# alexoz12v2/cuda-optix-pathtracing

Measured on AMD Instinct MI355X. Metric: Msamples/s (paths x spp / s), higher is better.
Workload: dtype f32

## Files before the change

### cuda-optix-pathtracing_amd/binding.py

```python
import ctypes as C
import subprocess
from pathlib import Path

import numpy as np

_HERE = Path(__file__).resolve().parent
_CSRC = _HERE / "csrc"
_LIB = None

DMT_ACCEL_BRUTE_FORCE = 0
DMT_ACCEL_BVH = 1
BVH_BUILD_HOST = 0
BVH_BUILD_DEVICE = 1
BVH_BUILT_BY_HOST = 0
BVH_BUILT_BY_DEVICE = 1
BVH_BUILT_BY_HOST_AFTER_DEVICE = 2
BVH_UPDATE_REBUILD = 0
BVH_UPDATE_REFIT = 1
BVH_UPDATE_AUTO = 2
BVH_UPDATED_NONE = 0
BVH_UPDATED_REFIT = 1
BVH_UPDATED_REBUILD = 2
BVH_UPDATED_REBUILD_AFTER_REFIT = 3

# ... 30 lines not shown
    return _LIB


EXPORTED_SYMBOLS = [
    "dmt_ctx_create", "dmt_ctx_destroy", "dmt_last_error", "dmt_upload_triangles", "dmt_upload_bsdfs",
    "dmt_upload_lights", "dmt_set_camera", "dmt_set_limits", "dmt_set_accel", "dmt_set_light_sampling", "dmt_light_tree_pmfs", "dmt_light_tree_ref_select", "dmt_set_bvh_strategy", "dmt_set_partition", "dmt_set_chunk", "dmt_render_profile",
    "dmt_upload_area_lights", "dmt_upload_textures", "dmt_upload_envmap", "dmt_clear_envmap", "dmt_envmap_tables", "dmt_test_envmap",
    "dmt_set_stream", "dmt_film_clear", "dmt_film_bind", "dmt_film_device_ptrs", "dmt_download_film",
    "dmt_render", "dmt_render_adaptive", "dmt_render_stats", "dmt_sync", "dmt_sched_diag", "dmt_kernel_time", "dmt_kernel_info", "dmt_bvh_validate", "dmt_brute_cull_plan", "dmt_brute_cull_box_plan", "dmt_brute_cull_box_records", "dmt_cull_box_test", "dmt_test_triangle_intersect",
    "dmt_test_sampler", "dmt_test_camera_rays", "dmt_test_bsdf", "dmt_test_bsdf_ng", "dmt_test_material", "dmt_test_light", "dmt_test_half",
    "dmt_test_trace_samples", "dmt_test_trace_log", "dmt_test_closest_hit",
    "dmt_set_texture_filter", "dmt_texture_mip_chain", "dmt_texture_footprint", "dmt_test_texture_filter",
    "dmt_render_aovs", "dmt_upload_aovs", "dmt_download_aovs", "dmt_denoise_defaults", "dmt_denoise",
    "dmt_set_accel_build", "dmt_accel_build_info", "dmt_accel_download", "dmt_lbvh_reference", "dmt_bvh_check",
    "dmt_update_vertices", "dmt_update_vertices_device", "dmt_set_accel_update", "dmt_accel_update_info", "dmt_bvh_refit_reference",
    "dmt_download_aov_surface", "dmt_upload_aov_surface", "dmt_camera_project", "dmt_test_camera_project", "dmt_temporal_defaults",
    "dmt_denoise_temporal", "dmt_temporal_reset", "dmt_temporal_info", "dmt_temporal_download",
    "dmt_set_sampler_table", "dmt_sampler_table_plan", "dmt_test_sampler_table",
    "dmt_set_lens", "dmt_lens_info", "dmt_lens_rays", "dmt_focus_distance_at", "dmt_test_lens_values",
    "dmt_set_motion", "dmt_clear_motion", "dmt_set_shutter", "dmt_motion_info", "dmt_shutter_times", "dmt_motion_positions",
    "dmt_motion_bvh_validate", "dmt_test_shutter_times", "dmt_test_closest_hit_at",
    "dmt_upload_vertex_normals", "dmt_clear_vertex_normals", "dmt_vertex_normals_info", "dmt_smooth_normals",
    "dmt_test_shading_normal", "dmt_test_shading_normal_mapped",
    "dmt_upload_opacity", "dmt_clear_opacity", "dmt_opacity_info", "dmt_opacity_eval", "dmt_test_opacity", "dmt_test_closest_hit_opacity",
]

SAMPLER_TABLE_OFF = 0
SAMPLER_TABLE_AUTO = 1
SAMPLER_TABLE_FORCE = 2


class SamplerTablePlanRecord(C.Structure):
    _fields_ = [("use", C.c_uint32), ("period_width", C.c_uint32), ("period_height", C.c_uint32), ("entry_bytes", C.c_uint32),
                ("slices", C.c_uint32), ("reserved", C.c_uint32), ("slice_bytes", C.c_uint64)]


def sampler_table_plan(width, height, owned_pixels, spp, chunk_spp, budget_bytes=0, mode=SAMPLER_TABLE_AUTO):
    lib = load_library()
    rec = SamplerTablePlanRecord()
    args = [int(width), int(height), C.c_uint64(int(owned_pixels)), C.c_uint32(int(spp)), C.c_uint32(int(chunk_spp)),
            C.c_uint64(int(budget_bytes)), int(mode)]
    rc = lib.dmt_sampler_table_plan(*args, C.byref(rec), None, C.c_uint32(0))
    if rc != 0:
        raise DmtError(f"dmt_sampler_table_plan failed ({rc})")
    lens = (C.c_uint32 * max(int(rec.slices), 1))()
    rc = lib.dmt_sampler_table_plan(*args, C.byref(rec), lens, C.c_uint32(int(rec.slices)))
# ... 579 lines not shown
        pairs = np.zeros((max(info["pairs"], 1), 2), np.uint32)
        self._check(self._lib.dmt_accel_download(self._ctx, _p(nodes), C.c_size_t(nodes.shape[0]), _p(pairs), C.c_size_t(pairs.shape[0])),
                    "dmt_accel_download")
        return nodes[:info["nodes"]].copy(), pairs[:info["pairs"]].copy()

    def set_light_sampling(self, mode):
        self._check(self._lib.dmt_set_light_sampling(self._ctx, int(mode)), "dmt_set_light_sampling")

    def set_texture_filter(self, mode):
        self._check(self._lib.dmt_set_texture_filter(self._ctx, int(mode)), "dmt_set_texture_filter")

    def set_bvh_strategy(self, strategy, paths_per_pass=0):
        self._check(self._lib.dmt_set_bvh_strategy(self._ctx, int(strategy), C.c_uint64(int(paths_per_pass))), "dmt_set_bvh_strategy")

    def set_partition(self, rank, world):
        self._check(self._lib.dmt_set_partition(self._ctx, int(rank), int(world)), "dmt_set_partition")

    def set_chunk(self, samples_per_item):
        self._check(self._lib.dmt_set_chunk(self._ctx, C.c_uint32(samples_per_item)), "dmt_set_chunk")

    def set_sampler_table(self, mode, budget_bytes=0):
        self._check(self._lib.dmt_set_sampler_table(self._ctx, int(mode), C.c_uint64(int(budget_bytes))), "dmt_set_sampler_table")

    def set_stream(self, stream_ptr):
        self._check(self._lib.dmt_set_stream(self._ctx, C.c_void_p(stream_ptr)), "dmt_set_stream")

    def film_clear(self):
        self._check(self._lib.dmt_film_clear(self._ctx), "dmt_film_clear")

    def film_bind(self, mean_ptr, m2_ptr):
        self._check(self._lib.dmt_film_bind(self._ctx, C.c_void_p(mean_ptr), C.c_void_p(m2_ptr)), "dmt_film_bind")

    def film_device_ptrs(self):
        a, b = C.c_void_p(), C.c_void_p()
        self._check(self._lib.dmt_film_device_ptrs(self._ctx, C.byref(a), C.byref(b)), "dmt_film_device_ptrs")
        return a.value, b.value

    def download_film(self):
        mean = np.zeros((self.height, self.width, 4), np.float32)
        m2 = np.zeros((self.height, self.width, 4), np.float32)
        self._check(self._lib.dmt_download_film(self._ctx, _p(mean), _p(m2)), "dmt_download_film")
        return mean, m2

    def render(self, spp, sample_offset=0, region=None):
        x0, y0, x1, y1 = region if region is not None else (0, 0, self.width, self.height)
        self._check(self._lib.dmt_render(self._ctx, C.c_uint32(sample_offset), C.c_uint32(spp), int(x0), int(y0),
# ... 100 lines not shown
        self._check(self._lib.dmt_temporal_info(self._ctx, C.byref(rec)), "dmt_temporal_info")
        return {name: getattr(rec, name) for name, _ in TemporalRecord._fields_}

    def download_history(self):
        cv = np.zeros((self.height, self.width, 4), np.float32)
        ln = np.zeros((self.height, self.width), np.float32)
        self._check(self._lib.dmt_temporal_download(self._ctx, _p(cv), _p(ln)), "dmt_temporal_download")
        return cv, ln

    def test_camera_project(self, points):
        p = _f32(points).reshape(-1, 3)
        xy, depth = np.zeros((p.shape[0], 2), np.float32), np.zeros(p.shape[0], np.float32)
        self._check(self._lib.dmt_test_camera_project(self._ctx, int(p.shape[0]), _p(p), _p(xy), _p(depth)), "dmt_test_camera_project")
        return xy, depth

    def sync(self):
        self._check(self._lib.dmt_sync(self._ctx), "dmt_sync")

    def sched_diag(self, reset=False):
        out = (C.c_uint64 * 8)()
        if not hasattr(self._lib, "dmt_sched_diag"):
            return dict.fromkeys(["folds", "handed_over", "folded_for_others", "slab_stalls", "early_exits",
                                  "max_stall_ticks_10ns", "launched", "slabs_per_wave"], 0)
        self._check(self._lib.dmt_sched_diag(self._ctx, out, int(bool(reset))), "dmt_sched_diag")
        keys = ["folds", "handed_over", "folded_for_others", "slab_stalls", "early_exits", "max_stall_ticks_10ns", "launched", "slabs_per_wave"]
        return dict(zip(keys, [int(x) for x in out]))

    def kernel_time(self, reset=True):
        ms, n = C.c_double(), C.c_uint64()
        self._check(self._lib.dmt_kernel_time(self._ctx, C.byref(ms), C.byref(n), int(bool(reset))), "dmt_kernel_time")
        return ms.value, n.value

    def kernel_info(self):
        v = [C.c_int() for _ in range(5)]
        self._check(self._lib.dmt_kernel_info(self._ctx, *[C.byref(x) for x in v]), "dmt_kernel_info")
        keys = ["vgprs", "sgprs", "lds_bytes", "blocks_per_cu", "cu_count"]
        return dict(zip(keys, (x.value for x in v)))

    def test_triangle_intersect(self, xs, ys, zs, o, d):
        xs, ys, zs = _f32(xs), _f32(ys), _f32(zs)
        n = xs.size // 4
        o, d = _f32(o), _f32(d)
        hit = np.zeros(n, np.int32)
        t = np.zeros(n, np.float32)
        pos, nrm, err = (np.zeros((n, 3), np.float32) for _ in range(3))
        self._check(self._lib.dmt_test_triangle_intersect(self._ctx, _p(xs), _p(ys), _p(zs), C.c_size_t(n), _p(o),
                                                          _p(d), _p(hit), _p(t), _p(pos), _p(nrm), _p(err)),
                    "dmt_test_triangle_intersect")
        return hit, t, pos, nrm, err
# ... 153 lines not shown
```

### cuda-optix-pathtracing_amd/csrc/dmt_hip.hip

```cpp
#include <hip/hip_runtime.h>

#include <algorithm>
#include <cassert>
#include <chrono>
#include <cmath>
#include <cstddef>
#include <cstdio>
#include <cstdlib>
#include <cstring>
#include <limits>
#include <map>
#include <memory>
#include <new>
#include <string>
#include <vector>

#include "../../include/dmt_hip.h"
#include "pt_device.hpp"
#include "bvh_device.hpp"
#include "bvh_gpu_build.hpp"
#include "devbuf.hpp"
#include "envmap.hpp"
#include "light_tree.hpp"
#include "light_tree_ref.hpp"
// ... 60 lines not shown
  int maxDepth;
  int shadeThreshold;
  EnvView env;
  uint32_t const* areaOf;
  uint32_t const* areaTri;
  float const* areaLe;
  uint32_t areaCount;
  uint32_t const* texRgba;
  int32_t const* texDesc;
  uint32_t const* matTex;
  float const* triUv;
  LightTreeNode const* lightTree;
  LightTreeRefNode const* lightTreeRef;
  unsigned long long* stats;
  float texCfr[12];
  float texMinDx[3], texMinDy[3];
  float texSppScale;
  uint32_t const* texMip;
  int32_t const* texMipDesc;
  MotionView motion;
  VtxNormalRec const* vtxNormals;
  OpacityRec const* opacity;
  float opacityCutoff8;
};

typedef RenderParams const DMT_CONST_AS* KArgs;
DMT_DEV KArgs kargs_base() { return (KArgs)__builtin_amdgcn_kernarg_segment_ptr(); }
DMT_DEV KArgs kargs(KArgs p) {
  asm volatile("" : "+s"(p));
  return p;
}
DMT_DEV SceneView load_scene(KArgs k) {
  k = kargs(k);
  SceneView s;
  s.tris = k->scene.tris, s.post = k->scene.post, s.bsdfs = k->scene.bsdfs, s.lights = k->scene.lights;
  s.infLights = k->scene.infLights, s.triCount = k->scene.triCount, s.bsdfCount = k->scene.bsdfCount;
  s.lightCount = k->scene.lightCount, s.infLightCount = k->scene.infLightCount;
  return s;
}
DMT_DEV BvhView load_bvh(KArgs k) {
  k = kargs(k);
  BvhView b;
  b.nodes = k->bvh.nodes, b.pairs = k->bvh.pairs, b.overflow = k->bvh.overflow, b.overflowStride = k->bvh.overflowStride;
  return b;
}

// ... 19 lines not shown
  unsigned long long const now = __builtin_readcyclecounter();
  unsigned long long const m = __ballot(1);
  if (int(__ffsll((long long)m)) - 1 == int(threadIdx.x & 63u)) {
    uint32_t const w = threadIdx.x >> 6;
    s_sectAcc[w][i] += now - s_sectLast[w];
    s_sectLast[w] = now;
  }
#endif
}
struct PathState {
  RayPair rp;
  f3 beta, L;
  int depth;
  bool lastT;
  bool active;
  bool hasShadow;
  bool finPending;
  float smax;
  Sampler rng;
  uint32_t sidx;
  float lastPdf;
  bool lastSpecular;
};
__shared__ float s_cold[7 * kLdsThreads];
DMT_DEV void put_C(f3 v) {
  float* const c = s_cold + threadIdx.x;
  c[0 * kLdsThreads] = v.x, c[1 * kLdsThreads] = v.y, c[2 * kLdsThreads] = v.z;
}
DMT_DEV f3 get_C() {
  float const* const c = s_cold + threadIdx.x;
  return mk3(c[0 * kLdsThreads], c[1 * kLdsThreads], c[2 * kLdsThreads]);
}
DMT_DEV void put_Lfin(f3 v) {
  float* const c = s_cold + threadIdx.x;
  c[3 * kLdsThreads] = v.x, c[4 * kLdsThreads] = v.y, c[5 * kLdsThreads] = v.z;
}
DMT_DEV f3 get_Lfin() {
  float const* const c = s_cold + threadIdx.x;
  return mk3(c[3 * kLdsThreads], c[4 * kLdsThreads], c[5 * kLdsThreads]);
}
DMT_DEV void put_finIdx(uint32_t i) { s_cold[6 * kLdsThreads + threadIdx.x] = __uint_as_float(i); }
DMT_DEV uint32_t get_finIdx() { return __float_as_uint(s_cold[6 * kLdsThreads + threadIdx.x]); }
DMT_DEV f3 ray_dir(PathState const& st) { return mk3(st.rp.dx.x, st.rp.dy.x, st.rp.dz.x); }
DMT_DEV f3 ray_org(PathState const& st) { return mk3(st.rp.ox.x, st.rp.oy.x, st.rp.oz.x); }
DMT_DEV void swap_rays(PathState& st) {
  auto sw = [](v2f& p) { float const t = p.x; p.x = p.y, p.y = t; };
// ... 993 lines not shown
template <bool STATS = false>
DMT_DEV void trace_pair_bvh(KArgs k, PathState const& st, bool doC, bool doS, uint32_t gtid, int& bestTri,
                            float& bu, float& bv, bool& occluded, LaneStats* ls = nullptr) {
  BvhView const bvh = load_bvh(k);
  float bt;
  if constexpr (STATS) ls->closest += doC ? 1u : 0u, ls->shadow += doS ? 1u : 0u;
  bvh_closest<STATS>(bvh, doC, mk3(st.rp.ox.x, st.rp.oy.x, st.rp.oz.x), mk3(st.rp.dx.x, st.rp.dy.x, st.rp.dz.x),
                     gtid, bestTri, bt, bu, bv, STATS ? &ls->tc : nullptr);
  occluded = bvh_any<STATS>(bvh, doS, mk3(st.rp.ox.y, st.rp.oy.y, st.rp.oz.y),
                            mk3(st.rp.dx.y, st.rp.dy.y, st.rp.dz.y), st.smax, gtid, STATS ? &ls->tc : nullptr);
}
DMT_DEV void trace_pair_bvh_motion(KArgs k, PathState const& st, bool doC, bool doS, v2f time, uint32_t gtid, int& bestTri, float& bu,
                                   float& bv, bool& occluded, float* btOut = nullptr) {
  BvhView const bvh = load_bvh(k);
  TriPairDelta const* const delta = kargs(k)->motion.pairDelta;
  float bt;
  bvh_closest<false>(bvh, doC, mk3(st.rp.ox.x, st.rp.oy.x, st.rp.oz.x), mk3(st.rp.dx.x, st.rp.dy.x, st.rp.dz.x), gtid, bestTri, bt, bu, bv,
                     nullptr, LeafMotion{delta, time.x});
  occluded = bvh_any<false>(bvh, doS, mk3(st.rp.ox.y, st.rp.oy.y, st.rp.oz.y), mk3(st.rp.dx.y, st.rp.dy.y, st.rp.dz.y), st.smax, gtid,
                            nullptr, LeafMotion{delta, time.y});
  if (btOut) *btOut = bt;
}

template <uint32_t F, class Sink>
DMT_DEV void lane_finish(KArgs k, PathState& st, bool doC, bool doS, int bestTri, float bu, float bv, bool occluded,
                         Sink&& sink);

template <uint32_t F, class Sink>
DMT_DEV void lane_step(KArgs k, uint32_t gtid, PathState& st, Sink&& sink, LaneStats* ls = nullptr) {
  bool const doC = st.active;
  bool const doS = st.hasShadow;
  int bestTri;
  float bu, bv;
  bool occluded;
  if constexpr ((F & kFeatCutout) && (F & kFeatBvh))
    trace_pair_bvh_cut(k, st, doC, doS, gtid, bestTri, bu, bv, occluded);
  else if constexpr (F & kFeatCutout)
    trace_pair_brute_cut(k, st, doC, doS, bestTri, bu, bv, occluded);
  else if constexpr ((F & kFeatMotion) && (F & kFeatBvh))
    trace_pair_bvh_motion(k, st, doC, doS, v2f{motion_time(), motion_time_shadow()}, gtid, bestTri, bu, bv, occluded);
  else if constexpr (F & kFeatMotion)
    trace_pair_brute_motion(k, st, doC, doS, v2f{motion_time(), motion_time_shadow()}, bestTri, bu, bv, occluded);
  else if constexpr (F & kFeatBvh)
    trace_pair_bvh<(F & kFeatStats) != 0>(k, st, doC, doS, gtid, bestTri, bu, bv, occluded, ls);
  else
    trace_pair_brute(k, st, doC, doS, bestTri, bu, bv, occluded);
  sect_mark(2);
  if constexpr (F & kFeatStats) ls->bounces += (doC && bestTri >= 0 && st.depth < kargs(k)->maxDepth) ? 1u : 0u;
  lane_finish<F & ~kFeatStats>(k, st, doC, doS, bestTri, bu, bv, occluded, sink);
}

template <uint32_t F, class Sink>
DMT_DEV void lane_finish(KArgs k, PathState& st, bool doC, bool doS, int bestTri, float bu, float bv, bool occluded,
                         Sink&& sink) {
  if (doS) {
    st.hasShadow = false;
    if (st.finPending) {
      f3 Lfin = get_Lfin();
      if (!occluded) Lfin = Lfin + get_C();
      st.finPending = false;
      sink(Lfin, get_finIdx());
    } else if (!occluded) {
      st.L = st.L + get_C();
    }
  }
  sect_mark(3);
  if (doC) {
    if (path_shade<F>(k, st, bestTri, bu, bv)) {
      st.active = false;
      if (st.hasShadow) {
        put_Lfin(st.L);
        put_finIdx(st.sidx);
        st.finPending = true;
      } else {
        sink(st.L, st.sidx);
      }
    }
  }
  if constexpr (F & kFeatMotion) {
    if (st.hasShadow) motion_park_shadow();
  }
  sect_mark(10);
}

__shared__ float s_prep[15 * kLdsThreads];

struct ColdArgs {
  CameraXf cam;
  SamplerParams sp;
// ... 103 lines not shown
  uint32_t* slabBusy;
  float* stage;
  int rank, world;
};
DMT_DEV TileArgs load_tile_args(KArgs k) {
  k = kargs(k);
  TileArgs t;
  t.mean = k->mean, t.m2 = k->m2, t.counter = k->counter, t.width = k->width;
  t.x0 = k->x0, t.y0 = k->y0, t.x1 = k->x1, t.y1 = k->y1, t.tx0 = k->tx0, t.ty0 = k->ty0, t.rtx = k->rtx;
  t.numItems = k->numItems, t.subShift = k->subShift, t.sampleOffset = k->sampleOffset, t.spp = k->spp, t.rank = k->rank, t.world = k->world;
  t.chunkSpp = k->chunkSpp, t.numChunks = k->numChunks, t.link = k->link, t.slabBusy = k->slabBusy, t.stage = k->stage;
  return t;
}

__shared__ uint32_t s_desc[kLdsThreads / 64][2][8];
__shared__ int32_t s_pixbase[2 * kLdsThreads];
__shared__ uint32_t s_pixmap[2 * kLdsThreads];

constexpr uint32_t kSlotBit = 0x80000000u;
constexpr uint32_t kFoldReady = 0xFFFFFFFFu;
#ifndef DMT_SLAB_WAIT_MS
#define DMT_SLAB_WAIT_MS 250
#endif
constexpr int kSchedDiagWords = 8;

struct WaveSched {
  uint32_t cur = 0, fetched = 0;
  uint32_t alloc = 0;
  uint32_t nextUnit = 0, totalUnits = 0;
  bool exhausted = false;
  uint32_t slabFree = (1u << kSlabsPerWave) - 1u;
  uint32_t slabPend = 0;
};
enum { SD_FOLDS = 0, SD_HANDED = 1, SD_CHAINED = 2, SD_STALLS = 3, SD_EXITS = 4, SD_MAXSTALL = 5 };
DMT_DEV void sched_count(unsigned long long* D, int lane, int what, unsigned long long n = 1ull) {
  if (lane == 0) atomicAdd(&D[what], n);
}
struct LaneSched {
  bool prepared = false;
  bool prepSlot = false;
};

struct ItemGeom {
  int px0, py0;
  uint32_t rows;
  unsigned long long live;
};
DMT_DEV ItemGeom item_geom(TileArgs const& T, uint32_t item) {
  uint32_t const band = item & ((1u << T.subShift) - 1u);
  uint32_t const rows = 8u >> T.subShift;
  uint32_t j;
  unsigned long long live = ~0ull;
  KArgs const k = kargs(kargs_base());
  if (uint32_t const* const list = k->tileList) {
    j = list[item >> T.subShift];
    live = kargs(k)->tileMask[j] >> (band * rows * 8u);
  } else {
// ... 221 lines not shown
      unsigned long long* const D = kargs(Pk)->schedDiag;
      sched_count(D, lane, SD_STALLS);
      unsigned long long const t0 = __builtin_amdgcn_s_memrealtime();
      unsigned long long waited = 0;
      do {
        __builtin_amdgcn_s_sleep(64);
        slab_refresh(T, gtid, lane, W);
        waited = __builtin_amdgcn_s_memrealtime() - t0;
      } while (W.slabFree == 0u && waited <= (unsigned long long)(DMT_SLAB_WAIT_MS) * 100000ull);
      if (lane == 0) atomicMax(&D[SD_MAXSTALL], waited);
      if (W.slabFree == 0u) {
        sched_count(D, lane, SD_EXITS);
        return false;
      }
    }
  }
  return true;
}
DMT_DEV bool lane_holds(PathState const& st, LaneSched const& Ls, bool curSlot) {
  return (st.active && ((st.sidx >> 31) != 0u) == curSlot) || (Ls.prepared && Ls.prepSlot == curSlot) ||
         (st.finPending && ((get_finIdx() >> 31) != 0u) == curSlot);
}

template <bool STATS>
DMT_DEV void flush_stats(KArgs Pk, LaneStats const& ls) {
  if constexpr (STATS) {
    unsigned long long* const stats = kargs(Pk)->stats;
    atomicAdd(&stats[0], (unsigned long long)ls.samples);
    atomicAdd(&stats[1], (unsigned long long)ls.closest);
    atomicAdd(&stats[2], (unsigned long long)ls.shadow);
    atomicAdd(&stats[3], (unsigned long long)ls.tc.nodes);
    atomicAdd(&stats[4], (unsigned long long)ls.tc.tris);
    atomicAdd(&stats[5], (unsigned long long)ls.bounces);
    atomicAdd(&stats[6], (unsigned long long)ls.itNode);
    atomicAdd(&stats[7], (unsigned long long)ls.itLeaf);
    atomicAdd(&stats[8], (unsigned long long)ls.itShade);
    atomicAdd(&stats[9], (unsigned long long)ls.itOuter);
    atomicAdd(&stats[10], (unsigned long long)ls.itPrep);
    atomicAdd(&stats[11], (unsigned long long)ls.lanesLeaf);
    atomicAdd(&stats[12], (unsigned long long)ls.lanesShade);
    atomicAdd(&stats[13], (unsigned long long)ls.lanesPrep);
    atomicAdd(&stats[14], (unsigned long long)ls.tc.deadNodes);
    atomicAdd(&stats[15], (unsigned long long)ls.tc.overflowPushes);
  }
}

template <uint32_t F>
DMT_DEV void megakernel_body() {
  static_assert(!(F & kFeatBvh), "BVH kernels run megakernel_body_bvh");
  constexpr bool STATS = (F & kFeatStats) != 0;
  constexpr bool MOTION = (F & kFeatMotion) != 0;
  KArgs const Pk = kargs_base();
  LaneStats ls;
  int const lane = int(threadIdx.x) & 63;
  uint32_t const gtid = blockIdx.x * blockDim.x + threadIdx.x;
  WaveSched W;
  LaneSched Ls;
  PathState st{};
  auto sink = [&](f3 L, uint32_t sidx) { stage_sample(Pk, sidx, L); };
#if DMT_SECTION_TIMING
  if (lane == 0) s_sectLast[threadIdx.x >> 6] = __builtin_readcyclecounter();
#endif
  if constexpr (!MOTION && !(F & kFeatCutout)) cull_stage(Pk);
#if DMT_SECTION_TIMING
  if (lane < 16) s_sectAcc[threadIdx.x >> 6][lane] = 0;
  sect_mark(15);
#endif
  {
    for (;;) {
      bool const needPrep = !Ls.prepared;
      bool const starving = !st.active && needPrep;
      if (__any(starving) || __popcll(__ballot(needPrep)) >= DMT_PREP_THRESHOLD) sched_draw<MOTION>(Pk, gtid, lane, W, Ls, needPrep);
      if (W.cur == W.fetched) break;
      if (!st.active && Ls.prepared) {
        path_begin_prepared<MOTION>(st);
        Ls.prepared = false;
        if constexpr (STATS) ++ls.samples;
      }
      sect_mark(0);
      if (W.alloc != W.cur || W.nextUnit == W.totalUnits) {
        if (!__any(lane_holds(st, Ls, (W.cur & 1u) != 0u))) {
          bool const more = sched_retire(Pk, gtid, lane, W);
          sect_mark(1);
          if (!more) break;
          continue;
        }
      }
      sect_mark(1);
      lane_step<F>(Pk, gtid, st, sink, STATS ? &ls : nullptr);
    }
  }
#if DMT_SECTION_TIMING
  if (lane < 16) atomicAdd(&g_sect[lane], s_sectAcc[threadIdx.x >> 6][lane]);
#endif
  flush_stats<STATS>(Pk, ls);
}

#ifndef DMT_BVH_NODE_WEIGHT
#define DMT_BVH_NODE_WEIGHT 1
#define DMT_BVH_LEAF_WEIGHT 2
#endif
#ifndef DMT_BVH_SHADE_THRESHOLD
#define DMT_BVH_SHADE_THRESHOLD 32
#endif
#ifndef DMT_BVH_DUMMY_LDS
#define DMT_BVH_DUMMY_LDS 0
#endif
template <uint32_t F>
DMT_DEV void megakernel_body_bvh() {
  static_assert((F & kFeatBvh) != 0, "brute-force kernels run megakernel_body");
  constexpr bool STATS = (F & kFeatStats) != 0;
  constexpr bool MOTION = (F & kFeatMotion) != 0;
  KArgs const Pk = kargs_base();
// ... 313 lines not shown
  DevBuf<float> d_env;
  EnvView env{};
  DevBuf<uint32_t> d_areaOf;
  DevBuf<uint32_t> d_areaTri;
  DevBuf<float> d_areaLe;
  uint32_t areaCount = 0;
  std::vector<uint32_t> h_areaTri;
  std::vector<float> h_areaLe;
  bool haveTris = false, haveBsdfs = false, haveLights = false, haveCamera = false;
  dmt_camera cam{};
  CameraXf xf{};
  SamplerParams sp{};
  float lensR = 0.f, lensD = 1.f;
  DevBuf<float4> ownMean, ownM2;
  float4* d_mean = nullptr;
  float4* d_m2 = nullptr;
  int filmW = 0, filmH = 0;
  DevBuf<uint32_t> d_counter;
  DevBuf<uint32_t> d_sched;
  DevBuf<unsigned long long> d_schedDiag;
  unsigned long long expectedFolds = 0;
  DevBuf<unsigned long long> d_stats;
  DevBuf<float> d_stage;
  DevBuf<float4> d_samTab;
  DevBuf<float2> d_samTabJit;
  DevBuf<float2> d_samTabLens;
  int samTabMode = DMT_SAMPLER_TABLE_AUTO;
  uint64_t samTabBudget = kSamTabDefaultBudget;
  DevBuf<unsigned long long> d_adMask;
  DevBuf<uint32_t> d_adList;
  DevBuf<uint32_t> d_adCount;
  DenoiseState dn;
  uint32_t chunkSpp = 0;
  int subShift = -1;
  int maxDepth = 32;
  int accel = DMT_ACCEL_BRUTE_FORCE;
  int rank = 0, world = 1;
  int cuCount = 0;
  std::vector<std::pair<hipEvent_t, hipEvent_t>> events;
  size_t eventsUsed = 0;
  double accumMs = 0.0;
  uint64_t accumLaunches = 0;
};

namespace {

// ... 464 lines not shown
    ctx->lightTreeNodes = uint32_t(nodes.size());
    ctx->lightTreeValid = true;
    return DMT_OK;
  }
  std::vector<light_tree::Item> items;
  for (uint32_t i = 0; i < ctx->lightCount; ++i) {
    light_tree::Item it{};
    if (!light_tree::itemOf(ctx->h_lights.data() + 32 * size_t(i), i, [](uint16_t h) { return h2f_host(h); }, it))
      return fail(ctx, DMT_ERR_STATE, "light tree: only point and spot lights can be in the light list");
    items.push_back(it);
  }
  std::vector<LightTreeNode> const nodes = light_tree::build(items, &ctx->lightTreeDepth);
  if (ctx->lightTreeDepth > 60) {
    ctx->lightTreeTooDeep = true;
    return DMT_OK;
  }
  HIP_TRY(ctx, ctx->d_lightTree.assign(nodes.data(), nodes.size()));
  ctx->lightTreeNodes = uint32_t(nodes.size());
  ctx->lightTreeValid = true;
  return DMT_OK;
}

int checkErrorFlag(dmt_ctx* ctx) {
  unsigned long long folds = 0;
  HIP_TRY(ctx, hipMemcpy(&folds, ctx->d_schedDiag.get(), sizeof(folds), hipMemcpyDeviceToHost));
  if (folds != ctx->expectedFolds) {
    char msg[200];
    snprintf(msg, sizeof(msg), "in-launch ordering: %llu sample chunks were folded into the film, %llu were launched: the film is invalid",
             folds, ctx->expectedFolds);
    ctx->expectedFolds = folds;
    return fail(ctx, DMT_ERR_HIP, msg);
  }
  return DMT_OK;
}

int finishTest(dmt_ctx* ctx) {
  HIP_TRY(ctx, hipGetLastError());
  HIP_TRY(ctx, hipStreamSynchronize(ctx->stream));
  return DMT_OK;
}

}

#include "denoise_host.hpp"

static int rebuildAreaLights(dmt_ctx* ctx);

extern "C" {
// ... 31 lines not shown
  }
  ctx->stream = ctx->ownStream;
  ctx->cuCount = prop.multiProcessorCount;
  ctx->ac.blocksPerCUBvh = bpcBvh > 0 ? bpcBvh : 1;
  if (char const* e3 = std::getenv("DMT_BVH_STRATEGY")) {
    int const v = std::atoi(e3);
    ctx->bvhStrategy = v < 0 || v > 2 ? 0 : v;
  }
  if (char const* e5 = std::getenv("DMT_BVH_SHADE_THRESHOLD")) {
    int const v = std::atoi(e5);
    ctx->ac.shadeThresholdEnv = v < 1 ? 0 : (v > 64 ? 64 : v);
  }
  if (char const* e4 = std::getenv("DMT_WF_PATHS")) {
    long long const v = std::atoll(e4);
    if (v >= 4096) ctx->wfTargetPaths = size_t(v);
  }
  if (char const* e6 = std::getenv("DMT_BRUTE_CULL")) {
    int const v = std::atoi(e6);
    ctx->bruteCull = v == 0 ? 0 : v == 1 ? 1 : 2;
  }
  if (char const* e7 = std::getenv("DMT_SAMPLER_TABLE")) {
    int const v = std::atoi(e7);
    ctx->samTabMode = v == 0 ? DMT_SAMPLER_TABLE_OFF : v == 2 ? DMT_SAMPLER_TABLE_FORCE : DMT_SAMPLER_TABLE_AUTO;
  }
  if (char const* e2 = std::getenv("DMT_SUB_SHIFT")) {
    int const v = std::atoi(e2);
    ctx->subShift = v < 0 ? -1 : (v > 2 ? 2 : v);
  }
  *out = ctx.release();
  return DMT_OK;
}

int dmt_ctx_destroy(dmt_ctx* ctx) {
  if (!ctx) return DMT_ERR_INVALID;
  (void)hipSetDevice(ctx->device);
  (void)hipStreamSynchronize(ctx->stream);
  for (auto& ev : ctx->events) {
    (void)hipEventDestroy(ev.first);
    (void)hipEventDestroy(ev.second);
  }
  if (ctx->ownStream) (void)hipStreamDestroy(ctx->ownStream);
  delete ctx;
  return DMT_OK;
}

const char* dmt_last_error(const dmt_ctx* ctx) { return ctx ? ctx->err.c_str() : g_createError.c_str(); }
// ... 360 lines not shown
  SamplerTablePlan tab;
  if (!stats6 && !wavefront && !sel && !(F & kFeatMotion))
    tab = samplerTablePlan(ctx->filmW, ctx->filmH, uint64_t(ownedTiles) * 64u, spp, P.chunkSpp, ctx->samTabBudget, ctx->samTabMode,
                           ctx->lensR > 0.f ? kSamTabLensEntryBytes : kSamTabEntryBytes);

  bool const useBvh = ctx->accel == DMT_ACCEL_BVH;
  uint32_t const wavesWanted = P.numItems * P.numChunks < P.numItems ? P.numItems : P.numItems * P.numChunks;
  uint32_t blocks = uint32_t(ctx->cuCount) * uint32_t(blocksPerCu);
  uint32_t const blocksNeeded = (wavesWanted + 3) / 4;
  if (blocks > blocksNeeded) blocks = blocksNeeded;
  if (blocks == 0) blocks = 1;

  if (ctx->eventsUsed == ctx->events.size()) {
    hipEvent_t a, b;
    HIP_TRY(ctx, hipEventCreate(&a));
    HIP_TRY(ctx, hipEventCreate(&b));
    ctx->events.emplace_back(a, b);
  }
  auto& ev = ctx->events[ctx->eventsUsed];
  {
    size_t const floats = size_t(blocks) * 4u * size_t(kSlabsPerWave) * size_t(P.chunkSpp) * 192u;
    HIP_TRY(ctx, ctx->d_stage.reserve(floats));
    P.stage = ctx->d_stage.get();
  }
  uint32_t const callChunks = P.numChunks;
  uint32_t const sliceChunks = tab.use ? tab.sliceChunks : callChunks;
  size_t const busyWords = size_t(blocks) * 4u * size_t(kSlabsPerWave);
  size_t const linkWords = sliceChunks > 1 ? size_t(P.numItems) * size_t(sliceChunks) : 0;
  {
    HIP_TRY(ctx, ctx->d_sched.reserve(busyWords + linkWords));
    P.slabBusy = ctx->d_sched.get(), P.link = ctx->d_sched.get() + busyWords;
    HIP_TRY(ctx, hipMemsetAsync(ctx->d_sched.get(), 0, (busyWords + linkWords) * sizeof(uint32_t), ctx->stream));
  }
  size_t const sliceEntries = size_t(std::min<uint64_t>(uint64_t(sliceChunks) * P.chunkSpp, spp)) * tab.pw * tab.ph;
  if (tab.use) {
    HIP_TRY(ctx, ctx->d_samTab.reserve(2 * sliceEntries));
    HIP_TRY(ctx, ctx->d_samTabJit.reserve(sliceEntries));
    P.samTab = ctx->d_samTab.get(), P.samTabJit = ctx->d_samTabJit.get(), P.samTabPw = tab.pw, P.samTabPh = tab.ph;
    if (ctx->lensR > 0.f) {
      HIP_TRY(ctx, ctx->d_samTabLens.reserve(sliceEntries));
      P.samTabLens = ctx->d_samTabLens.get();
    }
  }
  HIP_TRY(ctx, hipMemsetAsync(ctx->d_counter.get(), 0, sizeof(uint32_t), ctx->stream));
  HIP_TRY(ctx, hipEventRecord(ev.first, ctx->stream));
  uint64_t const launchFolds = uint64_t(P.numItems) * P.numChunks;
// ... 197 lines not shown
  if (!ctx || !stats16) return DMT_ERR_INVALID;
  if (ctx->accel != DMT_ACCEL_BVH) return fail(ctx, DMT_ERR_STATE, "dmt_render_profile: only the BVH path has device counters");
  return renderImpl(ctx, sample_offset, spp, x0, y0, x1, y1, stats16, 16);
}

int dmt_sync(dmt_ctx* ctx) {
  if (!ctx) return DMT_ERR_INVALID;
  HIP_TRY(ctx, hipSetDevice(ctx->device));
  HIP_TRY(ctx, hipStreamSynchronize(ctx->stream));
  return checkErrorFlag(ctx);
}

int dmt_sched_diag(dmt_ctx* ctx, uint64_t* out8, int reset) {
  if (!ctx || !out8) return DMT_ERR_INVALID;
  HIP_TRY(ctx, hipSetDevice(ctx->device));
  HIP_TRY(ctx, hipStreamSynchronize(ctx->stream));
  unsigned long long d[kSchedDiagWords] = {};
  HIP_TRY(ctx, hipMemcpy(d, ctx->d_schedDiag.get(), sizeof(d), hipMemcpyDeviceToHost));
  for (int i = 0; i < 8; ++i) out8[i] = i < kSchedDiagWords ? d[i] : 0;
  out8[6] = ctx->expectedFolds;
  out8[7] = uint64_t(kSlabsPerWave);
  if (reset) {
    HIP_TRY(ctx, hipMemset(ctx->d_schedDiag.get(), 0, sizeof(d)));
    ctx->expectedFolds = 0;
  }
  return DMT_OK;
}

static int rebuildAreaLights(dmt_ctx* ctx) {
  ctx->d_areaOf.reset(), ctx->d_areaTri.reset(), ctx->d_areaLe.reset(), ctx->areaCount = 0;
  uint32_t const n = uint32_t(ctx->h_areaTri.size());
  if (n == 0 || !ctx->haveTris) return DMT_OK;
  std::vector<uint32_t> of(ctx->triCount, 0xFFFFFFFFu);
  for (uint32_t k = 0; k < n; ++k) {
    if (ctx->h_areaTri[k] >= ctx->triCount) return fail(ctx, DMT_ERR_INVALID, "area light refers to a triangle outside the uploaded soup");
    of[ctx->h_areaTri[k]] = k;
  }
  DevBuf<uint32_t> areaOf, areaTri;
  DevBuf<float> areaLe;
  HIP_TRY(ctx, areaOf.assign(of.data(), of.size()));
  HIP_TRY(ctx, areaTri.assign(ctx->h_areaTri.data(), n));
  HIP_TRY(ctx, areaLe.assign(ctx->h_areaLe.data(), 3 * size_t(n)));
  ctx->d_areaOf = std::move(areaOf), ctx->d_areaTri = std::move(areaTri), ctx->d_areaLe = std::move(areaLe);
  ctx->areaCount = n;
  return DMT_OK;
}

int dmt_upload_area_lights(dmt_ctx* ctx, const uint32_t* triangle_index, const float* radiance_rgb, uint32_t count) {
// ... 427 lines not shown
```

### include/dmt_hip.h

```cpp
#ifndef DMT_HIP_H
#define DMT_HIP_H

#include <stddef.h>
#include <stdint.h>

#ifdef __cplusplus
extern "C" {
#endif

typedef struct dmt_ctx dmt_ctx;

typedef struct dmt_camera {
  float dir[3];
  float pos[3];
  int32_t width;
  int32_t height;
  int32_t spp;
  float focal_length;
  float sensor_size;
} dmt_camera;

enum {
  DMT_OK = 0,
  DMT_ERR_INVALID = 1,
// ... 85 lines not shown
  uint32_t entry_bytes;
  uint32_t slices;
  uint32_t reserved;
  uint64_t slice_bytes;
} dmt_sampler_table_plan_record;
int dmt_sampler_table_plan(int width, int height, uint64_t owned_pixels, uint32_t spp, uint32_t chunk_spp, uint64_t budget_bytes,
                           int mode, dmt_sampler_table_plan_record* out, uint32_t* slice_spp, uint32_t slice_cap);
int dmt_set_stream(dmt_ctx* ctx, void* hip_stream);

int dmt_film_clear(dmt_ctx* ctx);
int dmt_film_bind(dmt_ctx* ctx, void* d_mean, void* d_m2);
int dmt_film_device_ptrs(dmt_ctx* ctx, void** d_mean, void** d_m2);
int dmt_download_film(dmt_ctx* ctx, float* mean4, float* m24);

int dmt_render(dmt_ctx* ctx, uint32_t sample_offset, uint32_t spp, int x0, int y0, int x1, int y1);
int dmt_render_adaptive(dmt_ctx* ctx, uint32_t min_spp, uint32_t max_spp, uint32_t step_spp, float threshold,
                        int x0, int y0, int x1, int y1, uint32_t* rounds, uint64_t* samples);
int dmt_render_stats(dmt_ctx* ctx, uint32_t sample_offset, uint32_t spp, int x0, int y0, int x1, int y1,
                     uint64_t* stats6);
int dmt_render_profile(dmt_ctx* ctx, uint32_t sample_offset, uint32_t spp, int x0, int y0, int x1, int y1,
                       uint64_t* stats16);
int dmt_sync(dmt_ctx* ctx);
int dmt_sched_diag(dmt_ctx* ctx, uint64_t* out8, int reset);
int dmt_kernel_time(dmt_ctx* ctx, double* total_ms, uint64_t* launches, int reset);
int dmt_kernel_info(dmt_ctx* ctx, int* vgprs, int* sgprs, int* lds_bytes, int* blocks_per_cu,
                    int* cu_count);

int dmt_bvh_validate(const float* xs, const float* ys, const float* zs, size_t count, int* node_count,
                     int* depth, int* max_leaf);

enum {
  DMT_BVH_BUILD_HOST = 0,
  DMT_BVH_BUILD_DEVICE = 1,
};
enum {
  DMT_BVH_BUILT_BY_HOST = 0,
  DMT_BVH_BUILT_BY_DEVICE = 1,
  DMT_BVH_BUILT_BY_HOST_AFTER_DEVICE = 2,
};
int dmt_set_accel_build(dmt_ctx* ctx, int mode);
typedef struct dmt_accel_build_record {
  int32_t builder;
  int32_t depth;
  uint32_t triangles;
  uint32_t nodes;
  uint32_t pairs;
// ... 129 lines not shown
```

Measured before the change: 5860.

## Park GGX hits in a per-wave queue and shade them in coherent batches

Adds a per-wave global-memory queue where lanes that hit GGX dielectric or conductor materials park their path state (throughput, radiance, direction, hit, sampler dims). Lanes then refill with other paths, and the parked hits are resumed together once a threshold (default 32) is reached or the slab drains. The aim is to cut divergence in the costly microfacet shading branch so that more lanes of a wave run the same BSDF code at once. In exchange it adds extra global memory traffic for the spill and refill, more ballots and bookkeeping in the scheduler loop, and a consistency check that parked and resumed counts match. Only the plain brute-force kernel variant is affected.

```diff
diff --git a/cuda-optix-pathtracing_amd/binding.py b/cuda-optix-pathtracing_amd/binding.py
--- a/cuda-optix-pathtracing_amd/binding.py
+++ b/cuda-optix-pathtracing_amd/binding.py
@@ -76,6 +76,7 @@
     "dmt_motion_bvh_validate", "dmt_test_shutter_times", "dmt_test_closest_hit_at",
     "dmt_upload_vertex_normals", "dmt_clear_vertex_normals", "dmt_vertex_normals_info", "dmt_smooth_normals",
     "dmt_test_shading_normal", "dmt_test_shading_normal_mapped",
+    "dmt_set_ggx_batch", "dmt_ggx_batch_diag",
     "dmt_upload_opacity", "dmt_clear_opacity", "dmt_opacity_info", "dmt_opacity_eval", "dmt_test_opacity", "dmt_test_closest_hit_opacity",
 ]
 
@@ -701,6 +702,14 @@
     def set_sampler_table(self, mode, budget_bytes=0):
         self._check(self._lib.dmt_set_sampler_table(self._ctx, int(mode), C.c_uint64(int(budget_bytes))), "dmt_set_sampler_table")
 
+    def set_ggx_batch(self, batch):
+        self._check(self._lib.dmt_set_ggx_batch(self._ctx, C.c_uint32(int(batch))), "dmt_set_ggx_batch")
+
+    def ggx_batch(self):
+        out = (C.c_uint64 * 5)()
+        self._check(self._lib.dmt_ggx_batch_diag(self._ctx, out), "dmt_ggx_batch_diag")
+        return int(out[4])
+
     def set_stream(self, stream_ptr):
         self._check(self._lib.dmt_set_stream(self._ctx, C.c_void_p(stream_ptr)), "dmt_set_stream")
 
@@ -847,9 +856,14 @@
         if not hasattr(self._lib, "dmt_sched_diag"):
             return dict.fromkeys(["folds", "handed_over", "folded_for_others", "slab_stalls", "early_exits",
                                   "max_stall_ticks_10ns", "launched", "slabs_per_wave"], 0)
+        ggx = (C.c_uint64 * 5)()
+        if hasattr(self._lib, "dmt_ggx_batch_diag"):
+            self._check(self._lib.dmt_ggx_batch_diag(self._ctx, ggx), "dmt_ggx_batch_diag")
         self._check(self._lib.dmt_sched_diag(self._ctx, out, int(bool(reset))), "dmt_sched_diag")
         keys = ["folds", "handed_over", "folded_for_others", "slab_stalls", "early_exits", "max_stall_ticks_10ns", "launched", "slabs_per_wave"]
-        return dict(zip(keys, [int(x) for x in out]))
+        d = dict(zip(keys, [int(x) for x in out]))
+        d.update(ggx_parked=int(ggx[0]), ggx_resumed=int(ggx[1]), ggx_shade_passes=int(ggx[2]), ggx_shaded_full=int(ggx[3]))
+        return d
 
     def kernel_time(self, reset=True):
         ms, n = C.c_double(), C.c_uint64()
diff --git a/cuda-optix-pathtracing_amd/csrc/dmt_hip.hip b/cuda-optix-pathtracing_amd/csrc/dmt_hip.hip
--- a/cuda-optix-pathtracing_amd/csrc/dmt_hip.hip
+++ b/cuda-optix-pathtracing_amd/csrc/dmt_hip.hip
@@ -106,6 +106,8 @@
   VtxNormalRec const* vtxNormals;
   OpacityRec const* opacity;
   float opacityCutoff8;
+  uint32_t ggxBatchT;
+  float* ggxQueue;
 };
 
 typedef RenderParams const DMT_CONST_AS* KArgs;
@@ -171,6 +173,7 @@
   float lastPdf;
   bool lastSpecular;
 };
+DMT_DEV bool ggx_resumed(PathState const& st) { return st.depth < 0; }
 __shared__ float s_cold[7 * kLdsThreads];
 DMT_DEV void put_C(f3 v) {
   float* const c = s_cold + threadIdx.x;
@@ -1210,17 +1213,27 @@
   if (btOut) *btOut = bt;
 }
 
-template <uint32_t F, class Sink>
+struct NoPark {};
+template <uint32_t F, class Sink, class Park = NoPark>
 DMT_DEV void lane_finish(KArgs k, PathState& st, bool doC, bool doS, int bestTri, float bu, float bv, bool occluded,
-                         Sink&& sink);
-
-template <uint32_t F, class Sink>
-DMT_DEV void lane_step(KArgs k, uint32_t gtid, PathState& st, Sink&& sink, LaneStats* ls = nullptr) {
+                         Sink&& sink, Park&& park = Park{});
+
+template <uint32_t F, class Sink, class Park = NoPark>
+DMT_DEV void lane_step(KArgs k, uint32_t gtid, PathState& st, Sink&& sink, LaneStats* ls = nullptr, Park&& park = Park{}) {
+  constexpr bool PARK = !std::is_same<typename std::decay<Park>::type, NoPark>::value;
   bool const doC = st.active;
   bool const doS = st.hasShadow;
   int bestTri;
   float bu, bv;
   bool occluded;
+  if constexpr (PARK) {
+    static_assert(F == 0, "GGX batching: the plain brute-force row only");
+    trace_pair_brute(k, st, doC && !ggx_resumed(st), doS, bestTri, bu, bv, occluded);
+    if (ggx_resumed(st)) bestTri = __float_as_int(st.rp.ox.x), bu = st.rp.oy.x, bv = st.rp.oz.x;
+    sect_mark(2);
+    lane_finish<F>(k, st, doC, doS, bestTri, bu, bv, occluded, sink, park);
+    return;
+  }
   if constexpr ((F & kFeatCutout) && (F & kFeatBvh))
     trace_pair_bvh_cut(k, st, doC, doS, gtid, bestTri, bu, bv, occluded);
   else if constexpr (F & kFeatCutout)
@@ -1238,9 +1251,9 @@
   lane_finish<F & ~kFeatStats>(k, st, doC, doS, bestTri, bu, bv, occluded, sink);
 }
 
-template <uint32_t F, class Sink>
+template <uint32_t F, class Sink, class Park>
 DMT_DEV void lane_finish(KArgs k, PathState& st, bool doC, bool doS, int bestTri, float bu, float bv, bool occluded,
-                         Sink&& sink) {
+                         Sink&& sink, Park&& park) {
   if (doS) {
     st.hasShadow = false;
     if (st.finPending) {
@@ -1253,6 +1266,7 @@
     }
   }
   sect_mark(3);
+  if constexpr (!std::is_same<typename std::decay<Park>::type, NoPark>::value) doC = park(doC, bestTri, bu, bv);
   if (doC) {
     if (path_shade<F>(k, st, bestTri, bu, bv)) {
       st.active = false;
@@ -1402,7 +1416,7 @@
 #ifndef DMT_SLAB_WAIT_MS
 #define DMT_SLAB_WAIT_MS 250
 #endif
-constexpr int kSchedDiagWords = 8;
+constexpr int kSchedDiagWords = 12;
 
 struct WaveSched {
   uint32_t cur = 0, fetched = 0;
@@ -1412,7 +1426,8 @@
   uint32_t slabFree = (1u << kSlabsPerWave) - 1u;
   uint32_t slabPend = 0;
 };
-enum { SD_FOLDS = 0, SD_HANDED = 1, SD_CHAINED = 2, SD_STALLS = 3, SD_EXITS = 4, SD_MAXSTALL = 5 };
+enum { SD_FOLDS = 0, SD_HANDED = 1, SD_CHAINED = 2, SD_STALLS = 3, SD_EXITS = 4, SD_MAXSTALL = 5,
+       SD_GGX_PARKED = 8, SD_GGX_RESUMED = 9, SD_GGX_PASSES = 10, SD_GGX_FULL = 11 };
 DMT_DEV void sched_count(unsigned long long* D, int lane, int what, unsigned long long n = 1ull) {
   if (lane == 0) atomicAdd(&D[what], n);
 }
@@ -1680,6 +1695,88 @@
          (st.finPending && ((get_finIdx() >> 31) != 0u) == curSlot);
 }
 
+#ifndef DMT_GGX_BATCH_T
+#define DMT_GGX_BATCH_T 32
+#endif
+constexpr uint32_t kGgxQueueCap = 64;
+constexpr uint32_t kGgxFields = 24;
+struct GgxBatch {
+  uint32_t parked = 0;
+  uint32_t nParked = 0, nPasses = 0, nFull = 0;
+  DMT_DEV uint32_t queued() const { return (parked & 0xFFFFu) + (parked >> 16); }
+  DMT_DEV uint32_t of_slot(uint32_t slot) const { return (parked >> (slot * 16u)) & 0xFFFFu; }
+};
+DMT_DEV float* ggx_queue(KArgs Pk, uint32_t gtid, uint32_t slot) {
+  return kargs(Pk)->ggxQueue + (size_t(wave_index(gtid)) * (kGgxFields * kGgxQueueCap) + slot);
+}
+DMT_DEV uint32_t lane_rank(unsigned long long m) {
+  return __builtin_amdgcn_mbcnt_hi(uint32_t(m >> 32), __builtin_amdgcn_mbcnt_lo(uint32_t(m), 0u));
+}
+DMT_DEV bool ggx_park(KArgs Pk, uint32_t gtid, PathState& st, GgxBatch& G, bool doC, int bestTri, float bu, float bv) {
+  if (kargs(Pk)->ggxBatchT == 0u) return doC;
+  bool const resumed = ggx_resumed(st);
+  if (resumed) st.depth = ~st.depth;
+  bool ggx = false;
+  if (doC && !resumed && bestTri >= 0 && st.depth < kargs(Pk)->maxDepth) {
+    KArgs const k = kargs(Pk);
+    uint32_t const type = hi16(k->scene.bsdfs[k->scene.post[bestTri].matId].w[1]);
+    ggx = type == BS_GGX_DIEL || type == BS_GGX_COND;
+  }
+  unsigned long long const m = __ballot(ggx);
+  bool park = false;
+  if (m != 0ull) {
+    uint32_t const q = G.queued();
+    uint32_t const room = kGgxQueueCap - q;
+    uint32_t const want = uint32_t(__popcll(m));
+    uint32_t const n = want < room ? want : room;
+    uint32_t const rank = lane_rank(m);
+    park = ggx && rank < room;
+    if (park) {
+      float* const r = ggx_queue(Pk, gtid, q + rank);
+      float const* const u = s_sampler_u + threadIdx.x;
+      r[0 * kGgxQueueCap] = st.beta.x, r[1 * kGgxQueueCap] = st.beta.y, r[2 * kGgxQueueCap] = st.beta.z;
+      r[3 * kGgxQueueCap] = st.L.x, r[4 * kGgxQueueCap] = st.L.y, r[5 * kGgxQueueCap] = st.L.z;
+      r[6 * kGgxQueueCap] = st.rp.dx.x, r[7 * kGgxQueueCap] = st.rp.dy.x, r[8 * kGgxQueueCap] = st.rp.dz.x;
+      r[9 * kGgxQueueCap] = __int_as_float(bestTri), r[10 * kGgxQueueCap] = bu, r[11 * kGgxQueueCap] = bv;
+      r[12 * kGgxQueueCap] = __int_as_float(st.depth), r[13 * kGgxQueueCap] = __uint_as_float(st.sidx);
+      r[15 * kGgxQueueCap] = __uint_as_float(uint32_t(st.rng.dim) | (st.lastT ? 0x100u : 0u));
+#pragma unroll
+      for (uint32_t d = 0; d < 8; ++d) r[(16 + d) * kGgxQueueCap] = u[d * kLdsThreads];
+      st.active = false;
+    }
+    uint32_t const n1 = uint32_t(__popcll(__ballot(park && (st.sidx >> 31) != 0u)));
+    G.parked += (n - n1) + (n1 << 16), G.nParked += n, G.nFull += want - n;
+  }
+  if (__any(doC && (resumed || (ggx && !park)))) ++G.nPasses;
+  return doC && !park;
+}
+DMT_DEV void ggx_resume(KArgs Pk, uint32_t gtid, PathState& st, GgxBatch& G) {
+  uint32_t const q = G.queued();
+  unsigned long long const m = __ballot(!st.active);
+  if (m == 0ull) return;
+  uint32_t const have = uint32_t(__popcll(m));
+  uint32_t const n = have < q ? have : q;
+  uint32_t const rank = lane_rank(m);
+  bool const pop = !st.active && rank < q;
+  if (pop) {
+    float const* const r = ggx_queue(Pk, gtid, q - 1u - rank);
+    float* const u = s_sampler_u + threadIdx.x;
+    st.beta = mk3(r[0 * kGgxQueueCap], r[1 * kGgxQueueCap], r[2 * kGgxQueueCap]);
+    st.L = mk3(r[3 * kGgxQueueCap], r[4 * kGgxQueueCap], r[5 * kGgxQueueCap]);
+    st.rp.dx.x = r[6 * kGgxQueueCap], st.rp.dy.x = r[7 * kGgxQueueCap], st.rp.dz.x = r[8 * kGgxQueueCap];
+    st.rp.ox.x = r[9 * kGgxQueueCap], st.rp.oy.x = r[10 * kGgxQueueCap], st.rp.oz.x = r[11 * kGgxQueueCap];
+    st.depth = ~__float_as_int(r[12 * kGgxQueueCap]);
+    st.sidx = __float_as_uint(r[13 * kGgxQueueCap]);
+    uint32_t const flags = __float_as_uint(r[15 * kGgxQueueCap]);
+    st.rng.dim = int(flags & 0xFFu), st.lastT = (flags & 0x100u) != 0u;
+#pragma unroll
+    for (uint32_t d = 0; d < 8; ++d) u[d * kLdsThreads] = r[(16 + d) * kGgxQueueCap];
+    st.active = true;
+  }
+  uint32_t const n1 = uint32_t(__popcll(__ballot(pop && (st.sidx >> 31) != 0u)));
+  G.parked -= (n - n1) + (n1 << 16);
+}
+
 template <bool STATS>
 DMT_DEV void flush_stats(KArgs Pk, LaneStats const& ls) {
   if constexpr (STATS) {
@@ -1724,11 +1821,29 @@
   if (lane < 16) s_sectAcc[threadIdx.x >> 6][lane] = 0;
   sect_mark(15);
 #endif
+  constexpr bool BATCH = F == 0;
+  GgxBatch G;
   {
     for (;;) {
+      if constexpr (BATCH) {
+        uint32_t const q = G.queued();
+        if (q != 0u) {
+          uint32_t const ofCur = G.of_slot(W.cur & 1u);
+          bool const drain = W.nextUnit == W.totalUnits || (W.alloc != W.cur && ofCur != 0u);
+          if (drain || q >= kargs(Pk)->ggxBatchT) ggx_resume(Pk, gtid, st, G);
+        }
+      }
       bool const needPrep = !Ls.prepared;
       bool const starving = !st.active && needPrep;
-      if (__any(starving) || __popcll(__ballot(needPrep)) >= DMT_PREP_THRESHOLD) sched_draw<MOTION>(Pk, gtid, lane, W, Ls, needPrep);
+      if (__any(starving) || __popcll(__ballot(needPrep)) >= DMT_PREP_THRESHOLD) {
+        if constexpr (BATCH) {
+          int l = lane;
+          asm volatile("" : "+v"(l));
+          sched_draw<MOTION>(Pk, gtid, l, W, Ls, needPrep);
+        } else {
+          sched_draw<MOTION>(Pk, gtid, lane, W, Ls, needPrep);
+        }
+      }
       if (W.cur == W.fetched) break;
       if (!st.active && Ls.prepared) {
         path_begin_prepared<MOTION>(st);
@@ -1737,7 +1852,14 @@
       }
       sect_mark(0);
       if (W.alloc != W.cur || W.nextUnit == W.totalUnits) {
-        if (!__any(lane_holds(st, Ls, (W.cur & 1u) != 0u))) {
+        if constexpr (BATCH) {
+          if (G.of_slot(W.cur & 1u) == 0u && !__any(lane_holds(st, Ls, (W.cur & 1u) != 0u))) {
+            bool const more = sched_retire(Pk, gtid, lane, W);
+            sect_mark(1);
+            if (!more) break;
+            continue;
+          }
+        } else if (!__any(lane_holds(st, Ls, (W.cur & 1u) != 0u))) {
           bool const more = sched_retire(Pk, gtid, lane, W);
           sect_mark(1);
           if (!more) break;
@@ -1745,8 +1867,20 @@
         }
       }
       sect_mark(1);
-      lane_step<F>(Pk, gtid, st, sink, STATS ? &ls : nullptr);
-    }
+      if constexpr (BATCH)
+        lane_step<F>(Pk, gtid, st, sink, nullptr, [&](bool doC, int tri, float bu, float bv) {
+          return ggx_park(Pk, gtid, st, G, doC, tri, bu, bv);
+        });
+      else
+        lane_step<F>(Pk, gtid, st, sink, STATS ? &ls : nullptr);
+    }
+  }
+  if constexpr (BATCH) {
+    unsigned long long* const D = kargs(Pk)->schedDiag;
+    int const first = int(lane_rank(~0ull));
+    if (G.nParked != 0u) sched_count(D, first, SD_GGX_PARKED, G.nParked), sched_count(D, first, SD_GGX_RESUMED, G.nParked - G.queued());
+    if (G.nPasses != 0u) sched_count(D, first, SD_GGX_PASSES, G.nPasses);
+    if (G.nFull != 0u) sched_count(D, first, SD_GGX_FULL, G.nFull);
   }
 #if DMT_SECTION_TIMING
   if (lane < 16) atomicAdd(&g_sect[lane], s_sectAcc[threadIdx.x >> 6][lane]);
@@ -2106,6 +2240,9 @@
   unsigned long long expectedFolds = 0;
   DevBuf<unsigned long long> d_stats;
   DevBuf<float> d_stage;
+  DevBuf<float> d_ggxQueue;
+  uint32_t ggxBatchT = DMT_GGX_BATCH_T;
+  unsigned long long ggxLostReported = 0;
   DevBuf<float4> d_samTab;
   DevBuf<float2> d_samTabJit;
   DevBuf<float2> d_samTabLens;
@@ -2616,8 +2753,16 @@
 }
 
 int checkErrorFlag(dmt_ctx* ctx) {
-  unsigned long long folds = 0;
-  HIP_TRY(ctx, hipMemcpy(&folds, ctx->d_schedDiag.get(), sizeof(folds), hipMemcpyDeviceToHost));
+  unsigned long long d[kSchedDiagWords] = {};
+  HIP_TRY(ctx, hipMemcpy(d, ctx->d_schedDiag.get(), sizeof(d), hipMemcpyDeviceToHost));
+  unsigned long long const folds = d[SD_FOLDS];
+  if (d[SD_GGX_PARKED] - d[SD_GGX_RESUMED] != ctx->ggxLostReported) {
+    char msg[200];
+    snprintf(msg, sizeof(msg), "GGX batching: %llu hits were parked, %llu were taken back: the film is invalid", d[SD_GGX_PARKED],
+             d[SD_GGX_RESUMED]);
+    ctx->ggxLostReported = d[SD_GGX_PARKED] - d[SD_GGX_RESUMED];
+    return fail(ctx, DMT_ERR_HIP, msg);
+  }
   if (folds != ctx->expectedFolds) {
     char msg[200];
     snprintf(msg, sizeof(msg), "in-launch ordering: %llu sample chunks were folded into the film, %llu were launched: the film is invalid",
@@ -2695,6 +2840,10 @@
   if (char const* e7 = std::getenv("DMT_SAMPLER_TABLE")) {
     int const v = std::atoi(e7);
     ctx->samTabMode = v == 0 ? DMT_SAMPLER_TABLE_OFF : v == 2 ? DMT_SAMPLER_TABLE_FORCE : DMT_SAMPLER_TABLE_AUTO;
+  }
+  if (char const* e8 = std::getenv("DMT_GGX_BATCH")) {
+    int const v = std::atoi(e8);
+    ctx->ggxBatchT = v <= 0 ? 0u : std::min<uint32_t>(uint32_t(v), kGgxQueueCap);
   }
   if (char const* e2 = std::getenv("DMT_SUB_SHIFT")) {
     int const v = std::atoi(e2);
@@ -3101,6 +3250,10 @@
     size_t const floats = size_t(blocks) * 4u * size_t(kSlabsPerWave) * size_t(P.chunkSpp) * 192u;
     HIP_TRY(ctx, ctx->d_stage.reserve(floats));
     P.stage = ctx->d_stage.get();
+  }
+  if (ctx->ggxBatchT != 0u && F == 0u && !stats6 && !wavefront) {
+    HIP_TRY(ctx, ctx->d_ggxQueue.reserve(size_t(blocks) * size_t(kLdsThreads / 64) * size_t(kGgxFields) * size_t(kGgxQueueCap)));
+    P.ggxQueue = ctx->d_ggxQueue.get(), P.ggxBatchT = ctx->ggxBatchT;
   }
   uint32_t const callChunks = P.numChunks;
   uint32_t const sliceChunks = tab.use ? tab.sliceChunks : callChunks;
@@ -3344,8 +3497,25 @@
   out8[7] = uint64_t(kSlabsPerWave);
   if (reset) {
     HIP_TRY(ctx, hipMemset(ctx->d_schedDiag.get(), 0, sizeof(d)));
-    ctx->expectedFolds = 0;
-  }
+    ctx->expectedFolds = 0, ctx->ggxLostReported = 0;
+  }
+  return DMT_OK;
+}
+
+int dmt_set_ggx_batch(dmt_ctx* ctx, uint32_t batch) {
+  if (!ctx) return DMT_ERR_INVALID;
+  if (batch > kGgxQueueCap) return fail(ctx, DMT_ERR_INVALID, "dmt_set_ggx_batch: a batch is at most 64 hits (the queue's capacity)");
+  ctx->ggxBatchT = batch;
+  return DMT_OK;
+}
+
+int dmt_ggx_batch_diag(dmt_ctx* ctx, uint64_t* out5) {
+  if (!ctx || !out5) return DMT_ERR_INVALID;
+  HIP_TRY(ctx, hipSetDevice(ctx->device));
+  HIP_TRY(ctx, hipStreamSynchronize(ctx->stream));
+  unsigned long long d[kSchedDiagWords] = {};
+  HIP_TRY(ctx, hipMemcpy(d, ctx->d_schedDiag.get(), sizeof(d), hipMemcpyDeviceToHost));
+  out5[0] = d[SD_GGX_PARKED], out5[1] = d[SD_GGX_RESUMED], out5[2] = d[SD_GGX_PASSES], out5[3] = d[SD_GGX_FULL], out5[4] = ctx->ggxBatchT;
   return DMT_OK;
 }
 
diff --git a/include/dmt_hip.h b/include/dmt_hip.h
--- a/include/dmt_hip.h
+++ b/include/dmt_hip.h
@@ -131,6 +131,8 @@
                        uint64_t* stats16);
 int dmt_sync(dmt_ctx* ctx);
 int dmt_sched_diag(dmt_ctx* ctx, uint64_t* out8, int reset);
+int dmt_set_ggx_batch(dmt_ctx* ctx, uint32_t batch);
+int dmt_ggx_batch_diag(dmt_ctx* ctx, uint64_t* out5);
 int dmt_kernel_time(dmt_ctx* ctx, double* total_ms, uint64_t* launches, int reset);
 int dmt_kernel_info(dmt_ctx* ctx, int* vgprs, int* sgprs, int* lds_bytes, int* blocks_per_cu,
                     int* cu_count);
```

New measurement: 6110 (median of 6 runs). 1.04x the previous value.
